# Wionerlol/MultimodalEmotionRecognition

Measured on AMD Instinct MI355X. Metric: 3s-clip train steps/sec (B=32, xattn fusion) at 1/2/4/8 MI355X, higher is better.
Workload: dtype bf16; 1 GPU; ResNet18 + WavLM-base (frozen) + xattn fusion train step (fwd+bwd+Adam); per_gpu_batch=32, global_batch=32, frames=8, image=112, audio_samples=48000, parallelism=dp1

## Files before the change

multimodalemotionrecognition_amd/csrc/conv_wgrad.hip:

```cpp
#include "conv_common.h"
#include "mer.h"

MER_CT_BUFFER(mer_wct, 4096 * 8)
#define CTP(k) CTP_AT(mer_wct_buf, k)
MER_CT_MODE_WORD(mer_wct_mode)
#ifdef MER_CONV_TIMING
#define CT_MODE() mer_wct_mode_v
#else
#define CT_MODE() 0
#endif

namespace {

struct WgradGeom {
  int N, H, W, C;
  int Ho, Wo, K;
  int R, S, st, pad;
  int Creal;
  const bf16_t* X;
  const bf16_t* dY;
  float* ws;
  int pix_per_split;
  long ldy;
  int flat;
};

template <int BM_, int BN_, int WM = 2, int WN = 2, int PF = 1>
__global__ __launch_bounds__(64 * WM * WN, 2) void wgrad_kernel(WgradGeom g) {
  constexpr int NT = 64 * WM * WN;
  constexpr int LDM = BM_ + 16, LDN = BN_ + 16;
  constexpr int IT = BM_ / WM / 16, JT = BN_ / WN / 16;
  constexpr int ACH = BM_ * 64 / 8 / NT, BCH = BN_ * 64 / 8 / NT;
  static_assert(ACH * NT * 8 == BM_ * 64 && BCH * NT * 8 == BN_ * 64, "staging split");
  __shared__ __attribute__((aligned(16))) bf16_t lds[2][64 * LDM + 64 * LDN];
  const int t = threadIdx.x, lane = t & 63, w = t >> 6;
  const int Ntot = g.R * g.S * g.C;
  const int P = g.N * g.Ho * g.Wo;
  const int wnx = (Ntot + BN_ - 1) / BN_, wny = (g.K + BM_ - 1) / BM_;
  int wtx, wty;
  xcd_tile(blockIdx.x, wnx, wnx * wny, wtx, wty);
  const int m0 = wty * BM_, n0 = wtx * BN_;
  const int p_beg = blockIdx.z * g.pix_per_split, p_end = min(P, p_beg + g.pix_per_split);
  const int wm = (w / WN) * (BM_ / WM), wn = (w % WN) * (BN_ / WN);
  constexpr int ACPR = BM_ / 8, BCPR = BN_ / 8;

  u32x4 ra[ACH], rb[BCH], ra2[ACH], rb2[BCH];
  const int a_cc = t % ACPR, a_pr0 = t / ACPR;
  const int b_cc = t % BCPR, b_pr0 = t / BCPR;
  const int b_nn = n0 + b_cc * 8;
  const bool b_colok = b_nn < Ntot;
  const float inv_C = 1.f / g.C, inv_S = 1.f / g.S, inv_HoWo = 1.f / (g.Ho * g.Wo), inv_Wo = 1.f / g.Wo;
  const int b_tap = b_colok ? fdiv(b_nn, inv_C) : 0;
  const int b_c = b_colok ? b_nn - b_tap * g.C : 0;
  const int b_r = fdiv(b_tap, inv_S), b_s = b_tap - fdiv(b_tap, inv_S) * g.S;
  const int HoWo = g.Ho * g.Wo;
  unsigned okm = 0u, okm2 = 0u;
  auto gload = [&](u32x4* ra, u32x4* rb, unsigned& okm, int p0) {
    okm = 0u;
#pragma unroll
    for (int i = 0; i < ACH; ++i) {
      const int p = p0 + a_pr0 + i * (NT / ACPR), k = m0 + a_cc * 8;
      const bool ok = p < p_end && k < g.K;
      ra[i] = *reinterpret_cast<const u32x4*>(g.dY + (long)(p < p_end ? p : p_beg) * g.ldy + (k < g.K ? k : 0));
      okm |= (ok ? 1u : 0u) << i;
    }
#pragma unroll
    for (int i = 0; i < BCH; ++i) {
      const int p = p0 + b_pr0 + i * (NT / BCPR);
      const int pc = p < p_end ? p : p_beg;
      const int n = fdiv(pc, inv_HoWo);
      const int rem = pc - n * HoWo;
      const int oh = fdiv(rem, inv_Wo), ow = rem - oh * g.Wo;
      const int ih = oh * g.st - g.pad + b_r, iw = ow * g.st - g.pad + b_s;
      const bool ok = p < p_end && b_colok && ih >= 0 && ih < g.H && iw >= 0 && iw < g.W;
      const int ihc = ih < 0 ? 0 : (ih >= g.H ? g.H - 1 : ih), iwc = iw < 0 ? 0 : (iw >= g.W ? g.W - 1 : iw);
      rb[i] = *reinterpret_cast<const u32x4*>(g.X + (((long)n * g.H + ihc) * g.W + iwc) * g.C + b_c);
      okm |= (ok ? 1u : 0u) << (ACH + i);
    }
  };
  auto lstore = [&](int buf, const u32x4* ra, const u32x4* rb, unsigned okm) {
    const u32x4 z = {0u, 0u, 0u, 0u};
#pragma unroll
    for (int i = 0; i < ACH; ++i) {
      const int ch = t + NT * i;
      *reinterpret_cast<u32x4*>(&lds[buf][(ch / ACPR) * LDM + (ch % ACPR) * 8]) = ((okm >> i) & 1u) ? ra[i] : z;
    }
#pragma unroll
    for (int i = 0; i < BCH; ++i) {
      const int ch = t + NT * i;
      *reinterpret_cast<u32x4*>(&lds[buf][64 * LDM + (ch / BCPR) * LDN + (ch % BCPR) * 8]) =
          ((okm >> (ACH + i)) & 1u) ? rb[i] : z;
    }
  };
  auto tr_frag = [&](const bf16_t* img, int ld, int k0, int c0) -> bf16x8 {
    const int q = (lane & 15) >> 2, p4 = (lane & 3) * 4;
    const int kr = k0 + 8 * (lane >> 4);
    typedef __attribute__((address_space(3))) s16x4 lds_s16x4;
    const s16x4 lo = __builtin_amdgcn_ds_read_tr16_b64_v4i16((lds_s16x4*)(img + (kr + q) * ld + c0 + p4));
    const s16x4 hi = __builtin_amdgcn_ds_read_tr16_b64_v4i16((lds_s16x4*)(img + (kr + 4 + q) * ld + c0 + p4));
    typedef __attribute__((ext_vector_type(8))) short s16x8;
    s16x8 v = {lo[0], lo[1], lo[2], lo[3], hi[0], hi[1], hi[2], hi[3]};
    return __builtin_bit_cast(bf16x8, v);
  };

  f32x4 acc[IT][JT];
#pragma unroll
  for (int i = 0; i < IT; ++i)
#pragma unroll
    for (int j = 0; j < JT; ++j) acc[i][j] = f32x4{0.f, 0.f, 0.f, 0.f};

  const int nk = (p_end - p_beg + 63) / 64;
  auto compute = [&](int cur) {
    const bf16_t* Aimg = &lds[cur][0];
    const bf16_t* Bimg = &lds[cur][64 * LDM];
#pragma unroll
    for (int s = 0; s < 2; ++s) {
      bf16x8 af[IT], bfr[JT];
#pragma unroll
      for (int i = 0; i < IT; ++i) af[i] = tr_frag(Aimg, LDM, s * 32, wm + i * 16);
#pragma unroll
      for (int j = 0; j < JT; ++j) bfr[j] = tr_frag(Bimg, LDN, s * 32, wn + j * 16);
#pragma unroll
      for (int i = 0; i < IT; ++i)
#pragma unroll
        for (int j = 0; j < JT; ++j) acc[i][j] = __builtin_amdgcn_mfma_f32_16x16x32_bf16(af[i], bfr[j], acc[i][j], 0, 0, 0);
    }
  };
  if (PF == 1) {
    if (nk > 0) {
      gload(ra, rb, okm, p_beg);
      lstore(0, ra, rb, okm);
    }
    __syncthreads();
    for (int kt = 0; kt < nk; ++kt) {
      const int cur = kt & 1;
      gload(ra, rb, okm, p_beg + (kt + 1 < nk ? kt + 1 : kt) * 64);
      compute(cur);
      if (kt + 1 < nk) lstore(cur ^ 1, ra, rb, okm);
      __syncthreads();
    }
  } else {
    auto kstep = [&](int k) { return p_beg + (k < nk ? k : nk - 1) * 64; };
    if (nk > 0) {
      gload(ra, rb, okm, p_beg);
      gload(ra2, rb2, okm2, kstep(1));
      lstore(0, ra, rb, okm);
    }
    lds_barrier();
    for (int kt = 0; kt < nk; kt += 2) {
      gload(ra, rb, okm, kstep(kt + 2));
      compute(0);
      if (kt + 1 < nk) lstore(1, ra2, rb2, okm2);
      lds_barrier();
      if (kt + 1 >= nk) break;
      gload(ra2, rb2, okm2, kstep(kt + 3));
      compute(1);
      if (kt + 2 < nk) lstore(0, ra, rb, okm);
      lds_barrier();
    }
  }
  float* slab = g.ws + (long)blockIdx.z * g.K * Ntot;
#pragma unroll
  for (int i = 0; i < IT; ++i)
#pragma unroll
    for (int j = 0; j < JT; ++j) {
      const int nn = n0 + wn + j * 16 + (lane & 15);
      if (nn >= Ntot) continue;
#pragma unroll
      for (int rr = 0; rr < 4; ++rr) {
        const int k = m0 + wm + i * 16 + (lane >> 4) * 4 + rr;
        if (k < g.K) slab[(long)k * Ntot + nn] = acc[i][j][rr];
      }
    }
}


__device__ __forceinline__ int wswz(int row, int nchunks) { return ((row & 7) << 1) & (nchunks - 1); }

__device__ __forceinline__ s16x4 lds_read_tr16(const void* p) {
  typedef __attribute__((address_space(3))) const char lds_cchar;
  const uint32_t a = (uint32_t)(uintptr_t)(lds_cchar*)p;
  s16x4 v;
  asm volatile("ds_read_b64_tr_b16 %0, %1" : "=v"(v) : "v"(a) : "memory");
  return v;
}
template <int N>
__device__ __forceinline__ void lds_tr_wait() {
  asm volatile("s_waitcnt lgkmcnt(%0)" ::"n"(N) : "memory");
}
__device__ __forceinline__ void frag_ready(bf16x8& f) { asm volatile("" : "+v"(f)); }

template <int BM_, int BN_, int WM, int WN, int STAGES, int KS = 64, int KG = 1>
__global__ __launch_bounds__(64 * WM * WN * KG, KG > 1 ? WM * WN * KG / 4 : 2) void wgrad_pipe_kernel(WgradGeom g) {
  constexpr int WAVES = WM * WN;
  constexpr int ACW = BM_ / 8, BCW = BN_ / 8;
  constexpr int ARI = 64 / ACW, BRI = 64 / BCW;
  constexpr int IA = KS / ARI / WAVES, IB = KS / BRI / WAVES;
  static_assert(IA * ARI * WAVES == KS && IB * BRI * WAVES == KS, "the K-step must split into whole glds rows");
  static_assert(KS % 32 == 0, "MFMA k = 32 pixels");
  constexpr int IT = BM_ / WM / 16, JT = BN_ / WN / 16;
  constexpr int BUF = KS * (BM_ + BN_);
  extern __shared__ __attribute__((aligned(16))) bf16_t smem_all[];
  const int t = threadIdx.x, lane = t & 63, kg = (t >> 6) / WAVES, w = (t >> 6) % WAVES;
  CTP(0);
  bf16_t* const smem = smem_all + kg * STAGES * BUF;
  const int Ntot = g.R * g.S * g.C;
  const int P = g.N * g.Ho * g.Wo;
  const int wnx = (Ntot + BN_ - 1) / BN_, wny = (g.K + BM_ - 1) / BM_;
  int wtx, wty, zs;
  if (g.flat) {
    int tile;
    xcd_tile(blockIdx.x, wnx * wny, (int)gridDim.x, tile, zs);
    wty = tile / wnx;
    wtx = tile - wty * wnx;
  } else {
    xcd_tile(blockIdx.x, wnx, wnx * wny, wtx, wty);
    zs = blockIdx.z;
  }
  const int m0 = wty * BM_, n0 = wtx * BN_;
  const int p_beg = zs * g.pix_per_split, p_end = min(P, p_beg + g.pix_per_split);
  const int wm = (w / WN) * (BM_ / WM), wn = (w % WN) * (BN_ / WN);
  const bf16_t* zero = reinterpret_cast<const bf16_t*>(mer_conv_zero16);

  const int nk_all = (p_end - p_beg + KS - 1) / KS;
  const int nkg = (nk_all + KG - 1) / KG, kb = __builtin_amdgcn_readfirstlane(kg * nkg);
  const int nk = nk_all - kb < nkg ? (nk_all - kb > 0 ? nk_all - kb : 0) : nkg;
  const int pk0 = p_beg + kb * KS;

  const int HoWo = g.Ho * g.Wo;
  const bf16_t* ap[IA];
  int arow[IA];
  bool acok[IA];
#pragma unroll
  for (int j = 0; j < IA; ++j) {
    arow[j] = (w * IA + j) * ARI + lane / ACW;
    const int acol = m0 + ((lane % ACW) ^ wswz(arow[j], ACW)) * 8;
    acok[j] = acol < g.K;
    ap[j] = g.dY + ((long)(pk0 + arow[j]) * g.ldy + acol);
  }
  const long a_step = (long)KS * g.ldy;
  const bf16_t* bp[IB];
  int brow[IB], boh[IB], bow[IB], bdr[IB], bds[IB];
  bool bcok[IB];
#pragma unroll
  for (int j = 0; j < IB; ++j) {
    brow[j] = (w * IB + j) * BRI + lane / BCW;
    const int col = n0 + ((lane % BCW) ^ wswz(brow[j], BCW)) * 8;
    bcok[j] = col < Ntot;
    const int cc = bcok[j] ? col : 0;
    const int tap = cc / g.C, c = cc - tap * g.C;
    const int r = tap / g.S;
    bdr[j] = r - g.pad;
    bds[j] = tap - r * g.S - g.pad;
    const int p = pk0 + brow[j];
    const int n = p / HoWo, rem = p - n * HoWo;
    boh[j] = rem / g.Wo;
    bow[j] = rem - boh[j] * g.Wo;
    bp[j] = g.X + ((((long)n * g.H + boh[j] * g.st + bdr[j]) * g.W + bow[j] * g.st + bds[j]) * g.C + c);
  }
  const int s_dn = KS / HoWo, s_rem = KS - s_dn * HoWo, s_dh = s_rem / g.Wo, s_dw = s_rem - s_dh * g.Wo;
  const int d_step = ((s_dn * g.H + s_dh * g.st) * g.W + s_dw * g.st) * g.C;
  const int d_wrap_w = g.st * (g.W - g.Wo) * g.C;
  const int d_wrap_h = (g.H - g.Ho * g.st) * g.W * g.C;
  int p_left = p_end - pk0;
  auto stage = [&](int slot) {
    bf16_t* la = smem + slot * BUF;
    bf16_t* lb = la + KS * BM_;
#pragma unroll
    for (int j = 0; j < IA; ++j) {
      glds16(((int)(arow[j] < p_left) & (int)acok[j]) ? ap[j] : zero, la + (w * IA + j) * 512);
      ap[j] += a_step;
    }
#pragma unroll
    for (int j = 0; j < IB; ++j) {
      const int ok = (int)(brow[j] < p_left) & (int)bcok[j] &
                     (int)((unsigned)(__mul24(boh[j], g.st) + bdr[j]) < (unsigned)g.H) &
                     (int)((unsigned)(__mul24(bow[j], g.st) + bds[j]) < (unsigned)g.W);
      glds16(ok ? bp[j] : zero, lb + (w * IB + j) * 512);
      int d = d_step;
      bow[j] += s_dw;
      const bool cw = bow[j] >= g.Wo;
      bow[j] -= cw ? g.Wo : 0;
      d += cw ? d_wrap_w : 0;
      boh[j] += s_dh + (cw ? 1 : 0);
      const bool ch = boh[j] >= g.Ho;
      boh[j] -= ch ? g.Ho : 0;
      d += ch ? d_wrap_h : 0;
      bp[j] += d;
    }
    p_left -= KS;
  };
  auto tr_frag = [&](const bf16_t* img, int CW, int k0, int c0) -> bf16x8 {
    const int q = (lane & 15) >> 2, p4 = (lane & 3) * 4;
    const int kr = k0 + 8 * (lane >> 4);
    const int lc = (c0 + p4) >> 3, sub = (c0 + p4) & 7;
    const int r0 = kr + q, r1 = kr + 4 + q;
    const s16x4 lo = lds_read_tr16(img + r0 * CW * 8 + ((lc ^ wswz(r0, CW)) << 3) + sub);
    const s16x4 hi = lds_read_tr16(img + r1 * CW * 8 + ((lc ^ wswz(r1, CW)) << 3) + sub);
    typedef __attribute__((ext_vector_type(8))) short s16x8;
    s16x8 v = {lo[0], lo[1], lo[2], lo[3], hi[0], hi[1], hi[2], hi[3]};
    return __builtin_bit_cast(bf16x8, v);
  };

  f32x4 acc[IT][JT];
#pragma unroll
  for (int i = 0; i < IT; ++i)
#pragma unroll
    for (int j = 0; j < JT; ++j) acc[i][j] = f32x4{0.f, 0.f, 0.f, 0.f};
  constexpr int G = IA + IB;
#pragma unroll
  for (int s = 0; s < STAGES - 1; ++s)
    if (s < nk) stage(s);
  int wslot = STAGES - 1, rslot = 0;
#ifdef MER_CONV_TIMING
  bf16x8 af_h[KS / 32][IT] = {}, bfr_h[KS / 32][JT] = {};
#endif
  CTP(1);
  for (int kt = 0; kt < nkg; ++kt) {
    const int left = nk - 1 - kt;
    const int ahead = left < (STAGES - 2) ? left : (STAGES - 2);
    wait_tiles_in_flight<G>(ahead);
    lds_barrier();
    if (kt + STAGES - 1 < nk && CT_MODE() != 1) stage(wslot);
    wslot = wslot == STAGES - 1 ? 0 : wslot + 1;
    const bf16_t* Aimg = smem + rslot * BUF;
    rslot = rslot == STAGES - 1 ? 0 : rslot + 1;
    if (KG > 1 && kt >= nk) continue;
    const bf16_t* Bimg = Aimg + KS * BM_;
#pragma unroll
    for (int s = 0; s < KS / 32; ++s) {
      bf16x8 af[IT], bfr[JT];
#ifdef MER_CONV_TIMING
      if (CT_MODE() == 2 && kt > 0) {
#pragma unroll
        for (int i = 0; i < IT; ++i) af[i] = af_h[s][i];
#pragma unroll
        for (int j = 0; j < JT; ++j) bfr[j] = bfr_h[s][j];
      } else
#endif
      {
#pragma unroll
        for (int i = 0; i < IT; ++i) af[i] = tr_frag(Aimg, ACW, s * 32, wm + i * 16);
#pragma unroll
        for (int j = 0; j < JT; ++j) bfr[j] = tr_frag(Bimg, BCW, s * 32, wn + j * 16);
        lds_tr_wait<0>();
#pragma unroll
        for (int i = 0; i < IT; ++i) frag_ready(af[i]);
#pragma unroll
        for (int j = 0; j < JT; ++j) frag_ready(bfr[j]);
      }
#ifdef MER_CONV_TIMING
      if (kt == 0) {
#pragma unroll
        for (int i = 0; i < IT; ++i) af_h[s][i] = af[i];
#pragma unroll
        for (int j = 0; j < JT; ++j) bfr_h[s][j] = bfr[j];
      }
#endif
      __builtin_amdgcn_s_setprio(1);
#pragma unroll
      for (int i = 0; i < IT; ++i)
#pragma unroll
        for (int j = 0; j < JT; ++j) acc[i][j] = __builtin_amdgcn_mfma_f32_16x16x32_bf16(af[i], bfr[j], acc[i][j], 0, 0, 0);
      __builtin_amdgcn_s_setprio(0);
    }
  }
  CTP(2);
  if constexpr (KG > 1) {
    constexpr int LDR = BN_ + 4;
    __syncthreads();
    float* const part = reinterpret_cast<float*>(smem_all);
    if (kg > 0) {
      float* mine = part + (kg - 1) * BM_ * LDR;
#pragma unroll
      for (int i = 0; i < IT; ++i)
#pragma unroll
        for (int j = 0; j < JT; ++j)
#pragma unroll
          for (int rr = 0; rr < 4; ++rr)
            mine[(wm + i * 16 + (lane >> 4) * 4 + rr) * LDR + wn + j * 16 + (lane & 15)] = acc[i][j][rr];
    }
    lds_barrier();
    if (kg > 0) return;
#pragma unroll
    for (int i = 0; i < IT; ++i)
#pragma unroll
      for (int j = 0; j < JT; ++j)
#pragma unroll
        for (int rr = 0; rr < 4; ++rr)
#pragma unroll
          for (int q = 1; q < KG; ++q)
            acc[i][j][rr] += part[(q - 1) * BM_ * LDR + (wm + i * 16 + (lane >> 4) * 4 + rr) * LDR + wn + j * 16 +
                                  (lane & 15)];
  }
  CTP(3);
  float* slab = g.ws + (long)zs * g.K * Ntot;
#pragma unroll
  for (int i = 0; i < IT; ++i)
#pragma unroll
    for (int j = 0; j < JT; ++j) {
      const int nn = n0 + wn + j * 16 + (lane & 15);
      if (nn >= Ntot) continue;
#pragma unroll
      for (int rr = 0; rr < 4; ++rr) {
        const int k = m0 + wm + i * 16 + (lane >> 4) * 4 + rr;
        if (k < g.K) slab[(long)k * Ntot + nn] = acc[i][j][rr];
      }
    }
  CTP(4);
}

template <int BM_, int BN_, int WM, int WN, int STAGES, int KS = 64, int KG = 1>
int launch_wgrad_pipe(const WgradGeom& g0, dim3 grid, hipStream_t st) {
  const size_t ring = (size_t)KG * STAGES * KS * (BM_ + BN_) * sizeof(bf16_t);
  const size_t xchg = (size_t)(KG - 1) * BM_ * (BN_ + 4) * sizeof(float);
  const size_t lds = ring > xchg ? ring : xchg;
  if (hipFuncSetAttribute(reinterpret_cast<const void*>(&wgrad_pipe_kernel<BM_, BN_, WM, WN, STAGES, KS, KG>),
                          hipFuncAttributeMaxDynamicSharedMemorySize, (int)lds) != hipSuccess)
    return (int)hipErrorInvalidConfiguration;
  WgradGeom g = g0;
  g.flat = 1;
  const dim3 gr(grid.x * grid.z, 1, 1);
  hipLaunchKernelGGL((wgrad_pipe_kernel<BM_, BN_, WM, WN, STAGES, KS, KG>), gr, dim3(64 * WM * WN * KG), lds, st, g);
  return (int)hipSuccess;
}

struct StripGeom {
  int N, H, W, C, K;
  const bf16_t* X;
  const bf16_t* dY;
  float* ws;
  int ldy;
  int rows_per_split;
  int xrows;
};

__device__ __forceinline__ int sswz(int row, int nchunks) {
  return nchunks == 8 ? ((row & 2) | ((row >> 1) & 4)) : ((row >> 2) & 2);
}

struct StripUnit {
  const bf16_t* p;
  int n, h, w, u, lim, stride, wstride, dstep;
};

template <int KB, int STAGES>
__global__ __launch_bounds__(768, 3) void wgrad_strip_kernel(StripGeom g) {
  constexpr int KS = 64, NW = 12;
  constexpr int ACW = KB / 8;
  constexpr int ARI = 64 / ACW;
  constexpr int NDU = KS / ARI;
  constexpr int IT = KB / 16;
  constexpr int ABUF = KS * KB;
  static_assert(NDU >= NW - 8 && 8 + NDU <= 2 * NW, "8 X + NDU dY instructions over 12 waves, one or two each");
  static_assert(STAGES >= 2 && STAGES <= 4, "vmcnt waits below cover (STAGES - 2) * 2 <= 4");
  extern __shared__ __attribute__((aligned(16))) bf16_t smem_all[];
  bf16_t* const xring = smem_all;
  bf16_t* const aring = smem_all + g.xrows * 64;
  const int t = threadIdx.x, lane = t & 63, w = __builtin_amdgcn_readfirstlane(t >> 6);
  CTP(0);
  const int Wp = g.W + 1, Hp = g.H + 1, IQ = Hp * Wp, HL = Wp + 1;
  const int Ntot = 9 * g.C;
  const int nct = g.C / 64, ntile = nct * (g.K / KB);
  int tile, zs;
  xcd_tile(blockIdx.x, ntile, (int)gridDim.x, tile, zs);
  const int kti = tile / nct, cti = tile - kti * nct;
  const int k0 = kti * KB, c0 = cti * 64;
  const int TR = g.N * Hp;
  const int rb = zs * g.rows_per_split, re = min(TR, rb + g.rows_per_split);
  const int qb = rb * Wp, qlen = (re - rb) * Wp;
  const int nk = (qlen + KS - 1) / KS;
  const int NH = (2 * HL + KS - 1) / KS;
  const int xmask = g.xrows - 1;
  const bf16_t* zero = reinterpret_cast<const bf16_t*>(mer_conv_zero16);

  const int s_dn = KS / IQ, s_rem = KS - s_dn * IQ, s_dh = s_rem / Wp, s_dw = s_rem - s_dh * Wp;
  auto unit_init = [&](bool isx, int ui) -> StripUnit {
    StripUnit a;
    int row, chunk;
    if (isx) {
      row = ui * 8 + (lane >> 3);
      chunk = (lane & 7) ^ sswz(row, 8);
      a.stride = g.C;
      a.lim = qlen + 2 * HL;
    } else {
      row = ui * ARI + lane / ACW;
      chunk = (lane % ACW) ^ sswz(row, ACW);
      a.stride = g.ldy;
      a.lim = qlen;
    }
    const int qq = qb + row - (isx ? HL : 0) + IQ;
    const int n1 = qq / IQ, rem = qq - n1 * IQ;
    a.n = n1 - 1;
    a.h = rem / Wp;
    a.w = rem - a.h * Wp;
    a.u = row;
    a.wstride = g.W * a.stride;
    a.dstep = ((s_dn * g.H + s_dh) * g.W + s_dw) * a.stride;
    a.p = (isx ? g.X + c0 : g.dY + k0) + (((long)a.n * g.H + a.h) * g.W + a.w) * a.stride + chunk * 8;
    return a;
  };
  auto issue = [&](StripUnit& a, bf16_t* dst) {
    const int ok = (int)(a.u < a.lim) & (int)((unsigned)a.n < (unsigned)g.N) & (int)(a.h < g.H) & (int)(a.w < g.W);
    glds16(ok ? a.p : zero, dst);
    a.u += KS;
    int d = a.dstep;
    a.w += s_dw;
    const bool cw = a.w >= Wp;
    a.w -= cw ? Wp : 0;
    d -= cw ? a.stride : 0;
    a.h += s_dh + (cw ? 1 : 0);
    const bool ch = a.h >= Hp;
    a.h -= ch ? Hp : 0;
    d -= ch ? a.wstride : 0;
    a.n += s_dn + (ch ? 1 : 0);
    a.p += d;
  };
  const bool s0x = w < 8;
  const bool has1 = NDU > NW - 8 && w + NW - 8 < NDU;
  StripUnit u0 = unit_init(s0x, s0x ? w : w - 8);
  StripUnit u1 = unit_init(false, has1 ? w + NW - 8 : 0);
  int xw = 0;
  auto stage_x = [&]() {
    if (s0x) issue(u0, xring + (xw + w * 8) * 64);
    xw = (xw + KS) & xmask;
  };
  auto stage = [&](int aslot) {
    bf16_t* la = aring + aslot * ABUF;
    stage_x();
    if (!s0x) issue(u0, la + (w - 8) * 512);
    if (has1) issue(u1, la + (w + NW - 8) * 512);
  };

  const int g4 = lane >> 4, fq = (lane & 15) >> 2, p4 = (lane & 3) * 4;
  const int tr = w >> 2, cq = w & 3;
  int aoff[2][2][IT], xrow[3][2][2], xcol[3][2][2];
#pragma unroll
  for (int ss = 0; ss < 2; ++ss)
#pragma unroll
    for (int hi = 0; hi < 2; ++hi) {
      const int row = ss * 32 + 8 * g4 + 4 * hi + fq;
#pragma unroll
      for (int i = 0; i < IT; ++i) {
        const int col = i * 16 + p4;
        aoff[ss][hi][i] = (row * KB + ((((col >> 3) ^ sswz(row, ACW))) << 3) + (col & 7)) * 2;
      }
#pragma unroll
      for (int s = 0; s < 3; ++s) {
        const int xr = row + tr * Wp + s;
        const int col = cq * 16 + p4;
        xrow[s][ss][hi] = xr * 128;
        xcol[s][ss][hi] = (((((col >> 3) ^ sswz(xr, 8))) << 3) + (col & 7)) * 2;
      }
    }
  typedef __attribute__((ext_vector_type(8))) short s16x8;
  auto frag = [&](const char* lo_p, const char* hi_p) -> bf16x8 {
    const s16x4 lo = lds_read_tr16(lo_p);
    const s16x4 hi = lds_read_tr16(hi_p);
    s16x8 v = {lo[0], lo[1], lo[2], lo[3], hi[0], hi[1], hi[2], hi[3]};
    return __builtin_bit_cast(bf16x8, v);
  };

  f32x4 acc[3][IT];
#pragma unroll
  for (int s = 0; s < 3; ++s)
#pragma unroll
    for (int i = 0; i < IT; ++i) acc[s][i] = f32x4{0.f, 0.f, 0.f, 0.f};

  const char* const Xb = reinterpret_cast<const char*>(xring);
  auto read_frags = [&](int ss, const char* Ab, int xbB, bf16x8* af, bf16x8* bfr) {
#pragma unroll
    for (int i = 0; i < IT; ++i) af[i] = frag(Ab + aoff[ss][0][i], Ab + aoff[ss][1][i]);
#pragma unroll
    for (int s = 0; s < 3; ++s)
      bfr[s] = frag(Xb + (((xbB + xrow[s][ss][0]) & (g.xrows * 128 - 1)) + xcol[s][ss][0]),
                    Xb + (((xbB + xrow[s][ss][1]) & (g.xrows * 128 - 1)) + xcol[s][ss][1]));
    __builtin_amdgcn_sched_barrier(0);
  };
  constexpr int NFR = 2 * (IT + 3);
  auto frags_ready = [&](bf16x8* af, bf16x8* bfr) {
#pragma unroll
    for (int i = 0; i < IT; ++i) frag_ready(af[i]);
#pragma unroll
    for (int s = 0; s < 3; ++s) frag_ready(bfr[s]);
  };
  auto mfma_all = [&](const bf16x8* af, const bf16x8* bfr) {
    __builtin_amdgcn_s_setprio(1);
#pragma unroll
    for (int s = 0; s < 3; ++s)
#pragma unroll
      for (int i = 0; i < IT; ++i) acc[s][i] = __builtin_amdgcn_mfma_f32_16x16x32_bf16(af[i], bfr[s], acc[s][i], 0, 0, 0);
    __builtin_amdgcn_s_setprio(0);
    __builtin_amdgcn_sched_barrier(0);
  };
  bf16x8 af0[IT], bf0[3], af1[IT] = {}, bf1[3] = {};

  for (int pc = 0; pc < NH; ++pc) stage_x();
#pragma unroll
  for (int s = 0; s < STAGES - 1; ++s)
    if (s < nk) stage(s);
  int wslot = STAGES - 1, rslot = 0;
  const int xmaskB = g.xrows * 128 - 1;
  int xbB = 0;
  const int gw = has1 ? 2 : 1;
  CTP(1);
  for (int kt = 0; kt < nk; ++kt) {
    const int left = nk - 1 - kt;
    const int fly = (left < (STAGES - 2) ? left : (STAGES - 2)) * gw;
    if (fly <= 0) wait_vmcnt<0>();
    else if (fly == 1) wait_vmcnt<1>();
    else if (fly == 2) wait_vmcnt<2>();
    else wait_vmcnt<4>();
    lds_barrier();
    if (kt + STAGES - 1 < nk && CT_MODE() != 1) stage(wslot);
    wslot = wslot == STAGES - 1 ? 0 : wslot + 1;
    const char* Ab = reinterpret_cast<const char*>(aring + rslot * ABUF);
    rslot = rslot == STAGES - 1 ? 0 : rslot + 1;
    frags_ready(af1, bf1);
    if (CT_MODE() != 2 || kt == 0) read_frags(0, Ab, xbB, af0, bf0);
    mfma_all(af1, bf1);
    if (CT_MODE() != 2 || kt == 0) read_frags(1, Ab, xbB, af1, bf1);
    lds_tr_wait<NFR>();
    frags_ready(af0, bf0);
    mfma_all(af0, bf0);
    xbB = (xbB + KS * 128) & xmaskB;
  }
  lds_tr_wait<0>();
  frags_ready(af1, bf1);
  mfma_all(af1, bf1);
  CTP(2);
  CTP(3);
  float* slab = g.ws + (long)zs * g.K * Ntot;
#pragma unroll
  for (int s = 0; s < 3; ++s)
#pragma unroll
    for (int i = 0; i < IT; ++i) {
      const int nn = (tr * 3 + s) * g.C + c0 + cq * 16 + (lane & 15);
#pragma unroll
      for (int rr = 0; rr < 4; ++rr) slab[(long)(k0 + i * 16 + g4 * 4 + rr) * Ntot + nn] = acc[s][i][rr];
    }
  CTP(4);
}

template <int KB>
int launch_wgrad_strip(const WgradGeom& g0, int& splits, hipStream_t st) {
  constexpr int STAGES = 4;
  StripGeom g{};
  g.N = g0.N; g.H = g0.H; g.W = g0.W; g.C = g0.C; g.K = g0.K;
  g.X = g0.X; g.dY = g0.dY; g.ws = g0.ws; g.ldy = (int)g0.ldy;
  const int Wp = g.W + 1, Hp = g.H + 1;
  const long TR = (long)g.N * Hp;
  if (g0.ldy >= (1 << 24) || (TR + Hp) * Wp >= (1L << 30)) return (int)hipErrorInvalidValue;
  const int chunks = (2 * (Wp + 1) + 63) / 64 + STAGES;
  int xc = 1;
  while (xc < chunks) xc *= 2;
  if (xc > 8) return (int)hipErrorInvalidValue;
  g.xrows = xc * 64;
  if (splits < 1) splits = 1;
  g.rows_per_split = (int)((TR + splits - 1) / splits);
  splits = (int)((TR + g.rows_per_split - 1) / g.rows_per_split);
  const size_t lds = ((size_t)g.xrows * 64 + (size_t)STAGES * 64 * KB) * sizeof(bf16_t);
  if (hipFuncSetAttribute(reinterpret_cast<const void*>(&wgrad_strip_kernel<KB, STAGES>),
                          hipFuncAttributeMaxDynamicSharedMemorySize, (int)lds) != hipSuccess)
    return (int)hipErrorInvalidValue;
  const int tiles = (g.C / 64) * (g.K / KB);
  hipLaunchKernelGGL((wgrad_strip_kernel<KB, STAGES>), dim3(splits * tiles), dim3(768), lds, st, g);
  return (int)hipSuccess;
}

__global__ __launch_bounds__(256) void wgrad_reduce_kernel(int K, int C, int Creal, int RS, int splits, int SG,
                                                           float* __restrict__ ws) {
  __shared__ float part[256];
  const int E = 256 / SG, e = threadIdx.x % E, sg = threadIdx.x / E;
  const long total = (long)K * RS * C;
  const long idx = (long)blockIdx.x * E + e;
  float a0 = 0.f, a1 = 0.f, a2 = 0.f, a3 = 0.f;
  if (idx < total) {
    int z = sg;
    for (; z + 3 * SG < splits; z += 4 * SG) {
      a0 += ws[(long)z * total + idx];
      a1 += ws[(long)(z + SG) * total + idx];
      a2 += ws[(long)(z + 2 * SG) * total + idx];
      a3 += ws[(long)(z + 3 * SG) * total + idx];
    }
    for (; z < splits; z += SG) a0 += ws[(long)z * total + idx];
  }
  part[threadIdx.x] = (a0 + a1) + (a2 + a3);
  __syncthreads();
  if (sg != 0 || idx >= total) return;
  float s = 0.f;
  for (int q = 0; q < SG; ++q) s += part[q * E + e];
  ws[idx] = s;
}

__global__ __launch_bounds__(256) void wgrad_fold_scatter_kernel(int K, int C, int Creal, int RS, int splits,
                                                                 const float* __restrict__ ws, float* __restrict__ dw) {
  __shared__ float tile[49 * 32];
  const int k = blockIdx.y, c0 = blockIdx.x * 32;
  const long slab = (long)K * RS * C;
  const float* src = ws + (long)k * RS * C;
  for (int i = threadIdx.x; i < RS * 32; i += 256) {
    const int tap = i >> 5, c = c0 + (i & 31);
    const float* e = src + tap * C + (c < Creal ? c : 0);
    float s = 0.f;
    for (int z0 = 0; z0 < splits; z0 += 8) {
      float v[8];
#pragma unroll
      for (int q = 0; q < 8; ++q) v[q] = e[(long)(z0 + q < splits ? z0 + q : splits - 1) * slab];
#pragma unroll
      for (int q = 0; q < 8; ++q) s += z0 + q < splits ? v[q] : 0.f;
    }
    tile[i] = c < Creal ? s : 0.f;
  }
  __syncthreads();
  const int ncl = min(32, Creal - c0);
  const float inv_RS = 1.f / RS;
  float* dst = dw + ((long)k * Creal + c0) * RS;
  for (int i = threadIdx.x; i < ncl * RS; i += 256) {
    const int cl = fdiv(i, inv_RS), tap = i - cl * RS;
    dst[i] += tile[tap * 32 + cl];
  }
}

__global__ __launch_bounds__(256) void wgrad_scatter_kernel(int C, int Creal, int RS, const float* __restrict__ ws,
                                                            float* __restrict__ dw) {
  __shared__ float tile[49 * 32];
  const int k = blockIdx.y, c0 = blockIdx.x * 32;
  const float* src = ws + (long)k * RS * C;
  for (int i = threadIdx.x; i < RS * 32; i += 256) {
    const int tap = i >> 5, c = c0 + (i & 31);
    tile[i] = c < Creal ? src[tap * C + c] : 0.f;
  }
  __syncthreads();
  const int ncl = min(32, Creal - c0);
  const float inv_RS = 1.f / RS;
  float* dst = dw + ((long)k * Creal + c0) * RS;
  for (int i = threadIdx.x; i < ncl * RS; i += 256) {
    const int cl = fdiv(i, inv_RS), tap = i - cl * RS;
    dst[i] += tile[tap * 32 + cl];
  }
}

struct FoldRec {
  const float* ws;
  float* dw;
  const int* map;
  int K, C, Creal, RS, splits, SG, blk0, nblk;
};
constexpr int kFoldMaxRecs = 32;
struct FoldTable {
  int n;
  FoldRec r[kFoldMaxRecs];
};

__global__ __launch_bounds__(256) void wgrad_fold_batch_kernel(FoldTable t) {
  __shared__ f32x4 part[256];
  const int v = blockIdx.x;
  const int ri = table_find(t.n, v, [&](int i) { return t.r[i].blk0; });
  const FoldRec& R = t.r[ri];
  const int SG = R.SG, E = 256 / SG, e = threadIdx.x % E, sg = threadIdx.x / E;
  const long row = (long)R.RS * R.C, total = (long)R.K * row;
  const int lb = v - R.blk0;
  const long idx = ((long)lb * E + e) * 4;
  const f32x4 zero4 = {0.f, 0.f, 0.f, 0.f};
  f32x4 a0 = zero4, a1 = zero4, a2 = zero4, a3 = zero4;
  const int splits = R.splits;
  if (idx < total) {
    const f32x4* __restrict__ src = reinterpret_cast<const f32x4*>(R.ws + idx);
    const long st = total / 4;
    const int n = splits > sg ? (splits - sg + SG - 1) / SG : 0;
    for (int i0 = 0; i0 < n; i0 += 8) {
      f32x4 w[8];
#pragma unroll
      for (int q = 0; q < 8; ++q) {
        const int i = i0 + q < n ? i0 + q : n - 1;
        w[q] = src[(long)(sg + SG * i) * st];
      }
#pragma unroll
      for (int q = 0; q < 8; ++q)
        if (i0 + q < n) {
          if ((q & 3) == 0) a0 += w[q];
          else if ((q & 3) == 1) a1 += w[q];
          else if ((q & 3) == 2) a2 += w[q];
          else a3 += w[q];
        }
    }
  }
  part[threadIdx.x] = (a0 + a1) + (a2 + a3);
  __syncthreads();
  if (sg != 0 || idx >= total) return;
  f32x4 s4 = zero4;
  for (int q = 0; q < SG; ++q) s4 += part[q * E + e];
  const long per_k = R.map ? (long)R.Creal : (long)R.Creal * R.RS;
  const int k = (int)(idx / row), j0 = (int)(idx - (long)k * row);
  int o[4];
  float d[4];
  float* __restrict__ dwk = R.dw + (long)k * per_k;
#pragma unroll
  for (int c4 = 0; c4 < 4; ++c4) {
    const int j = j0 + c4;
    if (R.map) {
      o[c4] = R.map[j];
    } else {
      const int tap = j / R.C, c = j - tap * R.C;
      o[c4] = c < R.Creal ? c * R.RS + tap : -1;
    }
  }
#pragma unroll
  for (int c4 = 0; c4 < 4; ++c4) d[c4] = dwk[o[c4] >= 0 ? o[c4] : 0];
#pragma unroll
  for (int c4 = 0; c4 < 4; ++c4)
    if (o[c4] >= 0) dwk[o[c4]] = d[c4] + s4[c4];
}

}

MER_API int mer_conv_wgrad(int N, int H, int W, int C, int Creal, int K, int R, int S, int stride, int pad,
                           const void* x, const void* dy, float* dw, int splits, float* workspace, void* stream) {
  return mer_conv_wgrad_ex(N, H, W, C, Creal, K, R, S, stride, pad, x, dy, dw, splits, workspace, -1, stream);
}

static int conv_wgrad_impl(int N, int H, int W, int C, int Creal, int K, int R, int S, int stride, int pad,
                           const void* x, const void* dy, long ldy, float* dw, int splits, float* workspace,
                           int variant, void* stream, bool fold = true) {
  if (C % 8 || K % 8 || variant < -1 || variant > 10 || R * S > 49) return (int)hipErrorInvalidValue;
  if (variant == -1) variant = 4;
  const bool strip = variant == 9 || variant == 10;
  if (strip && (R != 3 || S != 3 || stride != 1 || pad != 1 || C % 64 || K % (variant == 9 ? 64 : 32) || Creal != C))
    return (int)hipErrorInvalidValue;
  WgradGeom g{};
  g.N = N; g.H = H; g.W = W; g.C = C; g.Creal = Creal;
  g.Ho = (H + 2 * pad - R) / stride + 1; g.Wo = (W + 2 * pad - S) / stride + 1; g.K = K;
  g.R = R; g.S = S; g.st = stride; g.pad = pad;
  g.X = (const bf16_t*)x; g.dY = (const bf16_t*)dy; g.ws = workspace;
  g.ldy = ldy > 0 ? ldy : K;
  const int P = N * g.Ho * g.Wo;
  const int splits_req = splits;
  if (splits < 1) splits = 1;
  g.pix_per_split = ((P + splits - 1) / splits + 63) / 64 * 64;
  splits = (P + g.pix_per_split - 1) / g.pix_per_split;
  const int Ntot = R * S * C;
  hipStream_t st = (hipStream_t)stream;
  int rc = (int)hipSuccess;
  if (strip) {
    splits = splits_req;
    rc = variant == 9 ? launch_wgrad_strip<64>(g, splits, st) : launch_wgrad_strip<32>(g, splits, st);
  } else if (K <= 64) {
    dim3 grid(((Ntot + 127) / 128) * ((K + 63) / 64), 1, splits);
    if (variant == 1)
      hipLaunchKernelGGL((wgrad_kernel<64, 128>), grid, dim3(256), 0, st, g);
    else if (variant == 4)
      rc = launch_wgrad_pipe<64, 128, 2, 4, 2>(g, grid, st);
    else if (variant == 8)
      rc = launch_wgrad_pipe<64, 128, 2, 4, 2, 64, 2>(g, grid, st);
    else if (variant == 5 || variant == 6)
      rc = launch_wgrad_pipe<64, 128, 2, 4, 3>(g, grid, st);
    else if (variant == 3)
      hipLaunchKernelGGL((wgrad_kernel<64, 128, 2, 4, 2>), grid, dim3(512), 0, st, g);
    else
      hipLaunchKernelGGL((wgrad_kernel<64, 128, 2, 4>), grid, dim3(512), 0, st, g);
  } else {
    dim3 grid(((Ntot + 127) / 128) * ((K + 127) / 128), 1, splits);
    if (variant == 1)
      hipLaunchKernelGGL((wgrad_kernel<128, 128>), grid, dim3(256), 0, st, g);
    else if (variant == 4)
      rc = launch_wgrad_pipe<128, 128, 2, 4, 2>(g, grid, st);
    else if (variant == 8)
      rc = launch_wgrad_pipe<128, 128, 2, 4, 2, 64, 2>(g, grid, st);
    else if (variant == 5)
      rc = launch_wgrad_pipe<128, 128, 2, 4, 3>(g, grid, st);
    else if (variant == 6)
      rc = launch_wgrad_pipe<128, 128, 2, 4, 4, 32>(g, grid, st);
    else if (variant == 7)
      rc = launch_wgrad_pipe<128, 128, 2, 4, 3, 32>(g, grid, st);
    else if (variant == 3)
      hipLaunchKernelGGL((wgrad_kernel<128, 128, 2, 4, 2>), grid, dim3(512), 0, st, g);
    else
      hipLaunchKernelGGL((wgrad_kernel<128, 128, 2, 4>), grid, dim3(512), 0, st, g);
  }
  if (rc != (int)hipSuccess) return rc;
  if (!fold) MER_LAUNCH_CHECK();
  constexpr int fold_max = 16;
  if (splits > fold_max) {
    const int SG = splits >= 64 ? 16 : 8;
    const long total = (long)K * R * S * C;
    const int E = 256 / SG;
    hipLaunchKernelGGL(wgrad_reduce_kernel, dim3((unsigned)((total + E - 1) / E)), dim3(256), 0, st, K, C, Creal, R * S,
                       splits, SG, workspace);
    hipLaunchKernelGGL(wgrad_scatter_kernel, dim3((Creal + 31) / 32, K), dim3(256), 0, st, C, Creal, R * S, workspace,
                       dw);
  } else {
    hipLaunchKernelGGL(wgrad_fold_scatter_kernel, dim3((Creal + 31) / 32, K), dim3(256), 0, st, K, C, Creal, R * S,
                       splits, workspace, dw);
  }
  MER_LAUNCH_CHECK();
}

MER_API int mer_conv_wgrad_ex(int N, int H, int W, int C, int Creal, int K, int R, int S, int stride, int pad,
                              const void* x, const void* dy, float* dw, int splits, float* workspace, int variant,
                              void* stream) {
  return conv_wgrad_impl(N, H, W, C, Creal, K, R, S, stride, pad, x, dy, K, dw, splits, workspace, variant, stream);
}

MER_API int mer_conv_wgrad_partials(int N, int H, int W, int C, int K, int R, int S, int stride, int pad,
                                    const void* x, const void* dy, int splits, float* workspace, int variant,
                                    void* stream) {
  return conv_wgrad_impl(N, H, W, C, C, K, R, S, stride, pad, x, dy, K, nullptr, splits, workspace, variant, stream,
                         false);
}

static int fold_sg_max() { return 8; }

MER_API int mer_wgrad_fold_batch(int n, const long long* rows, void* stream) {
  if (n < 1 || n > kFoldMaxRecs) return (int)hipErrorInvalidValue;
  FoldTable t{};
  t.n = n;
  int blk = 0;
  for (int i = 0; i < n; ++i) {
    const long long* q = rows + 8 * i;
    FoldRec& r = t.r[i];
    r.ws = (const float*)q[0]; r.dw = (float*)q[1]; r.map = (const int*)q[2];
    r.K = (int)q[3]; r.C = (int)q[4]; r.Creal = (int)q[5]; r.RS = (int)q[6]; r.splits = (int)q[7];
    if (!r.ws || !r.dw || r.K < 1 || r.C < 1 || r.C % 4 || r.RS < 1 || r.splits < 1 || r.Creal < 1 ||
        (!r.map && r.Creal > r.C) || ((uintptr_t)r.ws & 15))
      return (int)hipErrorInvalidValue;
    r.SG = r.splits > 48 ? fold_sg_max() : (r.splits > 12 ? 4 : 1);
    const long total = (long)r.K * r.RS * r.C;
    r.blk0 = blk;
    r.nblk = (int)((total + 4 * (256 / r.SG) - 1) / (4 * (256 / r.SG)));
    blk += r.nblk;
  }
  hipLaunchKernelGGL(wgrad_fold_batch_kernel, dim3(blk), dim3(256), 0, (hipStream_t)stream, t);
  MER_LAUNCH_CHECK();
}

MER_API int mer_linear_wgrad(int M, int N, int K, const void* x, const void* dy, long ldy, float* dw, int splits,
                             float* workspace, void* stream) {
  if (ldy < N || ldy % 8) return (int)hipErrorInvalidValue;
  return conv_wgrad_impl(1, 1, M, K, K, N, 1, 1, 1, 0, x, dy, ldy, dw, splits, workspace, -1, stream);
}
```

Baseline: 224.5 steps/s.

## Tile the wgrad split-fold via LDS transpose for coalesced dW writes

The batched wgrad fold kernel gains a tiled path for unmapped records. Each block handles one output channel k and a chunk of input channels, sums the split-K partials into an LDS tile, then writes the transposed (c, tap) layout of dw with vectorized, coalesced f32x4 read-modify-writes. The old path did scattered scalar stores. Host-side planning picks the chunk size and can flatten 1x1 records into 1024-wide rows. This adds template complexity and more LDS per block, which may lower occupancy.

```diff
diff --git a/multimodalemotionrecognition_amd/csrc/conv_wgrad.hip b/multimodalemotionrecognition_amd/csrc/conv_wgrad.hip
--- a/multimodalemotionrecognition_amd/csrc/conv_wgrad.hip
+++ b/multimodalemotionrecognition_amd/csrc/conv_wgrad.hip
@@ -746,25 +746,144 @@
   float* dw;
   const int* map;
   int K, C, Creal, RS, splits, SG, blk0, nblk;
+  int CC, chunks;
 };
 constexpr int kFoldMaxRecs = 32;
 struct FoldTable {
   int n;
   FoldRec r[kFoldMaxRecs];
 };
-
-__global__ __launch_bounds__(256) void wgrad_fold_batch_kernel(FoldTable t) {
-  __shared__ f32x4 part[256];
-  const int v = blockIdx.x;
-  const int ri = table_find(t.n, v, [&](int i) { return t.r[i].blk0; });
-  const FoldRec& R = t.r[ri];
-  const int SG = R.SG, E = 256 / SG, e = threadIdx.x % E, sg = threadIdx.x / E;
+constexpr int kFoldTile = 5120;
+constexpr int kFoldSlots = 5;
+constexpr int kFoldRunSG = 1016;
+
+template <int NB, int NEB, bool ONE>
+__device__ __forceinline__ void fold_tile_body(const float* __restrict__ src, long st, int C, int SG, int sg, int e,
+                                               int E, int n, int T4, int cw4, int CCp, float* part, int base) {
+  static_assert(NB % 4 == 0, "chain of slab i is i % 4");
+  const f32x4 zero4 = {0.f, 0.f, 0.f, 0.f};
+  const float inv_cw4 = 1.f / cw4;
+  int so[NEB], lo[NEB];
+#pragma unroll
+  for (int x = 0; x < NEB; ++x) {
+    const int q = base + x * E + e, qc = q < T4 ? q : 0;
+    const int tap = fdiv(qc, inv_cw4), c4 = qc - tap * cw4;
+    so[x] = tap * C + c4 * 4;
+    lo[x] = tap * CCp + c4 * 4;
+  }
+  f32x4 a[NEB][4];
+#pragma unroll
+  for (int x = 0; x < NEB; ++x)
+#pragma unroll
+    for (int c = 0; c < 4; ++c) a[x][c] = zero4;
+  int nv = n;
+  asm volatile("" : "+v"(nv));
+  auto batch = [&](int i0) {
+    f32x4 w[NEB][NB];
+#pragma unroll
+    for (int b = 0; b < NB; ++b) {
+      const int i = i0 + b < nv ? i0 + b : nv - 1;
+      const float* slab = src + (long)(__mul24(SG, i) + sg) * st;
+#pragma unroll
+      for (int x = 0; x < NEB; ++x) w[x][b] = *reinterpret_cast<const f32x4*>(slab + so[x]);
+    }
+#pragma unroll
+    for (int b = 0; b < NB; ++b)
+#pragma unroll
+      for (int x = 0; x < NEB; ++x) {
+        asm volatile("" : "+v"(w[x][b]));
+        if (i0 + b < nv) a[x][b & 3] += w[x][b];
+      }
+  };
+  if (n > 0) batch(0);
+  if (!ONE)
+    for (int i0 = NB; i0 < n; i0 += NB) batch(i0);
+#pragma unroll
+  for (int x = 0; x < NEB; ++x)
+    if (base + x * E + e < T4) *reinterpret_cast<f32x4*>(part + lo[x]) = (a[x][0] + a[x][1]) + (a[x][2] + a[x][3]);
+}
+
+template <int NB, bool ONE>
+__device__ __forceinline__ void fold_tile_sum(const float* __restrict__ src, long st, int C, int SG, int sg, int e,
+                                              int E, int n, int T4, int cw4, int CCp, float* part) {
+  constexpr int G = NB * 4 <= 16 ? 4 : (NB * 2 <= 16 ? 2 : 1);
+  int base = 0, ne = (T4 + E - 1) / E;
+#pragma unroll
+  for (int g = 0; g < kFoldSlots / G; ++g)
+    if (ne >= G) {
+      fold_tile_body<NB, G, ONE>(src, st, C, SG, sg, e, E, n, T4, cw4, CCp, part, base);
+      ne -= G, base += G * E;
+    }
+  if constexpr (G == 4)
+    if (ne >= 2) {
+      fold_tile_body<NB, 2, ONE>(src, st, C, SG, sg, e, E, n, T4, cw4, CCp, part, base);
+      ne -= 2, base += 2 * E;
+    }
+  if constexpr (G >= 2)
+    if (ne >= 1) fold_tile_body<NB, 1, ONE>(src, st, C, SG, sg, e, E, n, T4, cw4, CCp, part, base);
+}
+
+template <int NSLOT>
+__device__ __forceinline__ void fold_tiled(const FoldRec& R, int lb, float* lds) {
+  const int SG = R.SG, E = 256 / SG, tid = threadIdx.x, e = tid & (E - 1), sg = tid / E;
+  const int RS = R.RS, k = lb / R.chunks, c0 = (lb - k * R.chunks) * R.CC;
+  const int cw = min(R.CC, ((R.Creal + 3) & ~3) - c0), cw4 = cw >> 2, CCp = R.CC + 4;
+  const int L = min(cw, R.Creal - c0) * RS;
+  float* __restrict__ dst = R.dw + ((long)k * R.Creal + c0) * RS;
+  const int head = min((4 - (int)(((uintptr_t)dst >> 2) & 3)) & 3, L), nb = (L - head) >> 2, tail0 = head + 4 * nb;
+  const int ei = tid < 3 ? tid : tail0 + tid - 3;
+  const bool edge = tid < 3 ? tid < head : (tid < 6 && ei < L);
+  const long row = (long)RS * R.C, total = (long)R.K * row;
+  const float* src = R.ws + (long)k * row + c0;
+  const float* dwv = nb > 0 ? dst + head : src;
+  f32x4 d[NSLOT];
+#pragma unroll
+  for (int j = 0; j < NSLOT; ++j) d[j] = *reinterpret_cast<const f32x4*>(dwv + 4 * min(tid + 256 * j, max(nb - 1, 0)));
+  const float de = dst[edge ? ei : 0];
+  const int splits = R.splits, n = splits > sg ? (splits - sg + SG - 1) / SG : 0, T4 = RS * cw4;
+  float* part = lds + sg * RS * CCp;
+  if (NSLOT == 1) fold_tile_sum<8, false>(src, total, R.C, SG, sg, e, E, n, T4, cw4, CCp, part);
+  else if (splits <= 4) fold_tile_sum<4, true>(src, total, R.C, 1, 0, e, E, n, T4, cw4, CCp, part);
+  else if (splits <= 8) fold_tile_sum<8, true>(src, total, R.C, 1, 0, e, E, n, T4, cw4, CCp, part);
+  else fold_tile_sum<12, true>(src, total, R.C, 1, 0, e, E, n, T4, cw4, CCp, part);
+  __syncthreads();
+  const float inv_RS = 1.f / RS;
+  auto sum_at = [&](int i) {
+    const int cl = fdiv(i, inv_RS), tap = i - cl * RS;
+    float s = 0.f;
+    for (int q = 0; q < SG; ++q) s += lds[(q * RS + tap) * CCp + cl];
+    return s;
+  };
+#pragma unroll
+  for (int j = 0; j < NSLOT; ++j)
+    if (tid + 256 * j < nb) {
+      const int i = head + 4 * (tid + 256 * j);
+      f32x4 r;
+#pragma unroll
+      for (int x = 0; x < 4; ++x) r[x] = d[j][x] + sum_at(i + x);
+      *reinterpret_cast<f32x4*>(dst + i) = r;
+    }
+  if (edge) dst[ei] = de + sum_at(ei);
+}
+
+__device__ __forceinline__ void fold_source(const FoldRec& R, int lb, f32x4* part) {
+  const int SG = R.SG, E = 256 / SG, e = threadIdx.x & (E - 1), sg = threadIdx.x / E;
   const long row = (long)R.RS * R.C, total = (long)R.K * row;
-  const int lb = v - R.blk0;
   const long idx = ((long)lb * E + e) * 4;
   const f32x4 zero4 = {0.f, 0.f, 0.f, 0.f};
   f32x4 a0 = zero4, a1 = zero4, a2 = zero4, a3 = zero4;
   const int splits = R.splits;
+  const bool writer = sg == 0 && idx < total;
+  const int k = (int)(idx / row), j0 = (int)(idx - (long)k * row);
+  float* __restrict__ dwk = R.dw + (long)k * R.Creal;
+  int o[4] = {-1, -1, -1, -1};
+  float d[4] = {0.f, 0.f, 0.f, 0.f};
+  if (writer) {
+#pragma unroll
+    for (int c4 = 0; c4 < 4; ++c4) o[c4] = R.map[j0 + c4];
+#pragma unroll
+    for (int c4 = 0; c4 < 4; ++c4) d[c4] = dwk[o[c4] >= 0 ? o[c4] : 0];
+  }
   if (idx < total) {
     const f32x4* __restrict__ src = reinterpret_cast<const f32x4*>(R.ws + idx);
     const long st = total / 4;
@@ -788,29 +907,22 @@
   }
   part[threadIdx.x] = (a0 + a1) + (a2 + a3);
   __syncthreads();
-  if (sg != 0 || idx >= total) return;
+  if (!writer) return;
   f32x4 s4 = zero4;
   for (int q = 0; q < SG; ++q) s4 += part[q * E + e];
-  const long per_k = R.map ? (long)R.Creal : (long)R.Creal * R.RS;
-  const int k = (int)(idx / row), j0 = (int)(idx - (long)k * row);
-  int o[4];
-  float d[4];
-  float* __restrict__ dwk = R.dw + (long)k * per_k;
-#pragma unroll
-  for (int c4 = 0; c4 < 4; ++c4) {
-    const int j = j0 + c4;
-    if (R.map) {
-      o[c4] = R.map[j];
-    } else {
-      const int tap = j / R.C, c = j - tap * R.C;
-      o[c4] = c < R.Creal ? c * R.RS + tap : -1;
-    }
-  }
-#pragma unroll
-  for (int c4 = 0; c4 < 4; ++c4) d[c4] = dwk[o[c4] >= 0 ? o[c4] : 0];
 #pragma unroll
   for (int c4 = 0; c4 < 4; ++c4)
     if (o[c4] >= 0) dwk[o[c4]] = d[c4] + s4[c4];
+}
+
+__global__ __launch_bounds__(256) void wgrad_fold_batch_kernel(FoldTable t) {
+  __shared__ __attribute__((aligned(16))) float lds[kFoldTile];
+  const int v = blockIdx.x;
+  const int ri = table_find(t.n, v, [&](int i) { return t.r[i].blk0; });
+  const FoldRec& R = t.r[ri];
+  if (R.map) fold_source(R, v - R.blk0, reinterpret_cast<f32x4*>(lds));
+  else if (R.SG > 1) fold_tiled<1>(R, v - R.blk0, lds);
+  else fold_tiled<kFoldSlots>(R, v - R.blk0, lds);
 }
 
 }
@@ -927,7 +1039,26 @@
     r.SG = r.splits > 48 ? fold_sg_max() : (r.splits > 12 ? 4 : 1);
     const long total = (long)r.K * r.RS * r.C;
     r.blk0 = blk;
-    r.nblk = (int)((total + 4 * (256 / r.SG) - 1) / (4 * (256 / r.SG)));
+    if (r.map) {
+      r.nblk = (int)((total + 4 * (256 / r.SG) - 1) / (4 * (256 / r.SG)));
+    } else {
+      if (r.RS == 1 && r.Creal == r.C && r.C < 1024 && total % 1024 == 0) {
+        r.K = (int)(total / 1024);
+        r.C = r.Creal = 1024;
+      }
+      const int E = 256 / r.SG, cr4 = (r.Creal + 3) & ~3;
+      int cap = (kFoldTile / (r.SG * r.RS) - 4) & ~3;
+      if (r.SG > 1) cap = std::min(cap, (kFoldRunSG / r.RS) & ~3);
+      if (cap < 4) return (int)hipErrorInvalidValue;
+      int cc = cr4;
+      if (r.SG > 1)
+        for (cc = 32; r.RS * cc / 4 < E && cc < cr4;) cc *= 2;
+      cc = std::min(std::min(cc, cr4), cap);
+      if (cc > 32) cc &= ~31;
+      r.CC = cc;
+      r.chunks = (cr4 + cc - 1) / cc;
+      r.nblk = r.K * r.chunks;
+    }
     blk += r.nblk;
   }
   hipLaunchKernelGGL(wgrad_fold_batch_kernel, dim3(blk), dim3(256), 0, (hipStream_t)stream, t);
```

Measured after the change: 228.3 steps/s (median of 6 runs). 1.7% higher.
